# GenomicBreeding/GenomicBreedingModels.jl

Measured on AMD Instinct MI355X. Metric: GRM+GBLUP genotype-cells/s (n x p), higher is better.
Workload: dtype f64

## Files before the change

### genomicbreedingmodels.jl_amd/csrc/chol.hip

```cpp
#include <cstdlib>
#include <string>

#include "chol_device.h"

namespace gbm {

constexpr int NB = kCholNB;
constexpr int MAXRHS = 63;

int launch_chol_update(double* G, int64_t ldg, int64_t k0, int64_t nb, int64_t gdim, double* Ld, double* Dinv,
                       int32_t* info, int64_t next_k0, int rank, int nranks, hipStream_t s, int64_t col_lo = 0,
                       int64_t col_hi = INT64_MAX, int64_t row_lo = 0, int64_t row_hi = INT64_MAX);
int launch_chol_row_update(double* G, int64_t ldg, int64_t k0, int kch, int64_t gdim, double* Ld, double* Dinv,
                           int32_t* info, hipStream_t s, ColKeep keep = ColKeep{});
int64_t chol_small_lim();
void chol_refresh_tuning();
int64_t chol_flow_flag_bytes(int64_t gdim);
bool chol_flow_enabled(int64_t npad);
int launch_chol_flow(double* G, int64_t ldg, int64_t gdim, double* Ld, double* Dinv, void* flag_block, int32_t* info,
                     hipStream_t s);

__global__ void __launch_bounds__(256) prepare_v_kernel(double* __restrict__ G, int64_t ld, int64_t n,
                                                        int64_t npad, int64_t gdim, double inv_q,
                                                        const int64_t* __restrict__ q_dev, double lambda,
// ... 199 lines not shown
    if (area && j == c) {
#pragma unroll
      for (int m = 0; m < 2; m++)
#pragma unroll
        for (int q = 0; q < 2; q++)
#pragma unroll
          for (int r = 0; r < 4; r++) {
            int64_t row, col;
            quad(m, q, r, row, col);
            G[(r0 + row) * ld + jx + col] = accd[m][q][r];
            Us[row * PS + col] = accd[m][q][r];
          }
      __syncthreads();
      const int bad = factor_diag_block(Us, rinv, tid);
      if (tid == 0 && bad >= 0) atomicCAS(info, 0, (int32_t)(r0 + bad + 1));
      const __amdgpu_buffer_rsrc_t rL = wt_rsrc(Ld + r0 * CNB, CNB * CNB * 8);
      const __amdgpu_buffer_rsrc_t rD = wt_rsrc(Dinv + (r0 / 16) * 256, 1024 * 8);
      store_factor_with(
          Us, rinv, tid, [&](int e, wt_d2 v) { wt_st2(rL, (uint32_t)(e * 8), v); },
          [&](int e, double x) { wt_st1(rD, (uint32_t)(e * 8), x); });
      publish_flag(&prog[c], j + 1, tid);
      break;
    }
    {
      const double* src = G + r0 * ld + jx;
#pragma unroll
      for (int m = 0; m < 2; m++)
#pragma unroll
        for (int q = 0; q < 2; q++)
#pragma unroll
          for (int r = 0; r < 4; r++) {
            int64_t row, col;
            quad(m, q, r, row, col);
            acc[m][q][r] = src[row * ld + col];
          }
    }
    int seen = j == 0 ? 1 : 0;
    auto need = [&](int32_t v) -> bool {
      if (seen >= v) return true;
      __syncthreads();
      if (tid == 0) {
        s_ok = wait_flag<false>(&prog[j], v, info) ? 1 : 0;
        s_seen = __hip_atomic_load(&prog[j], __ATOMIC_RELAXED, __HIP_MEMORY_SCOPE_AGENT);
      }
      __syncthreads();
      seen = s_seen;
      return s_ok != 0;
    };
    if (j > 0) {
      d16 va, vb;
      auto load_step = [&](int i) {
        const __amdgpu_buffer_rsrc_t rk = wt_rsrc(G + (k0 + (int64_t)i * CNB) * ld, slab);
#pragma unroll
        for (int e = 0; e < 8; e++) {
          const int64_t rowoff = (int64_t)(lrow + 8 * e) * ld;
          const wt_d2 x = wt_ld2(rk, (uint32_t)((rowoff + r0 + lcol) * 8));
          const wt_d2 y = wt_ld2(rk, (uint32_t)((rowoff + jx + lcol) * 8));
          va[2 * e] = x.x;
          va[2 * e + 1] = x.y;
          vb[2 * e] = y.x;
          vb[2 * e + 1] = y.y;
        }
      };
      if (!need(1)) return;
      load_step(0);
      for (int i = 0; i < j; i++) {
        if (i > 0) __syncthreads();
#pragma unroll
        for (int e = 0; e < 8; e++) {
          *reinterpret_cast<wt_d2*>(&As[(lrow + 8 * e) * PS + lcol]) = (wt_d2){va[2 * e], va[2 * e + 1]};
          *reinterpret_cast<wt_d2*>(&Bs[(lrow + 8 * e) * PS + lcol]) = (wt_d2){vb[2 * e], vb[2 * e + 1]};
        }
        __syncthreads();
        if (i + 1 < j) {
          if (!need(i + 2)) return;
          load_step(i + 1);
        }
#pragma unroll
        for (int ks = 0; ks < 16; ks++) {
          double af[2], bf[2];
#pragma unroll
          for (int m = 0; m < 2; m++) af[m] = -As[(ks * 4 + fr) * PS + wm * 32 + m * 16 + fc];
#pragma unroll
          for (int q = 0; q < 2; q++) bf[q] = Bs[(ks * 4 + fr) * PS + wn * 32 + q * 16 + fc];
#pragma unroll
          for (int m = 0; m < 2; m++)
#pragma unroll
            for (int q = 0; q < 2; q++) acc[m][q] = __builtin_amdgcn_mfma_f64_16x16x4f64(af[m], bf[q], acc[m][q], 0, 0, 0);
        }
      }
      if (!need(j + 1)) return;
    }
    __syncthreads();
    double di[16];
#pragma unroll
    for (int m = 0; m < 2; m++)
#pragma unroll
      for (int q = 0; q < 2; q++)
#pragma unroll
        for (int r = 0; r < 4; r++) {
          int64_t row, col;
          quad(m, q, r, row, col);
          X[row * PS + col] = acc[m][q][r];
        }
    {
      const __amdgpu_buffer_rsrc_t rL = wt_rsrc(Ld + r0 * CNB, CNB * CNB * 8);
      const __amdgpu_buffer_rsrc_t rD = wt_rsrc(Dinv + (r0 / 16) * 256, 1024 * 8);
      wt_d2 u[8];
#pragma unroll
      for (int k = 0; k < 8; k++) u[k] = wt_ld2(rL, (uint32_t)((2 * tid + 512 * k) * 8));
#pragma unroll
      for (int rb = 0; rb < 4; rb++)
#pragma unroll
        for (int ks = 0; ks < 4; ks++) di[rb * 4 + ks] = wt_ld1(rD, (uint32_t)((rb * 256 + (ks * 4 + fr) * 16 + fc) * 8));
#pragma unroll
      for (int k = 0; k < 8; k++) {
        const int e = 2 * tid + 512 * k;
        *reinterpret_cast<wt_d2*>(&Us[(e >> 6) * PS + (e & 63)]) = u[k];
      }
    }
    __syncthreads();
    panel_chunk_solve(X, Us, [&](int rb, int ks) { return di[rb * 4 + ks]; }, lane, wave);
    __syncthreads();
#pragma unroll
    for (int e = 0; e < 8; e++) {
      const int row = lrow + 8 * e;
      wt_st2(rrow, (uint32_t)(((int64_t)row * ld + jx + lcol) * 8), *reinterpret_cast<const wt_d2*>(&X[row * PS + lcol]));
    }
#pragma unroll
    for (int e = 0; e < 8; e++) {
      const int row = lrow + 8 * e;
      *reinterpret_cast<double2*>(G + (jx + row) * ld + r0 + lcol) = make_double2(X[lcol * PS + row], X[(lcol + 1) * PS + row]);
    }
    if (area) {
#pragma unroll
      for (int ks = 0; ks < 16; ks++) {
        double af[2], bf[2];
#pragma unroll
        for (int m = 0; m < 2; m++) af[m] = -X[(ks * 4 + fr) * PS + wm * 32 + m * 16 + fc];
#pragma unroll
        for (int q = 0; q < 2; q++) bf[q] = X[(ks * 4 + fr) * PS + wn * 32 + q * 16 + fc];
#pragma unroll
        for (int m = 0; m < 2; m++)
#pragma unroll
          for (int q = 0; q < 2; q++) accd[m][q] = __builtin_amdgcn_mfma_f64_16x16x4f64(af[m], bf[q], accd[m][q], 0, 0, 0);
      }
      publish_flag(&prog[c], j + 1, tid);
    } else {
      __syncthreads();
    }
  }
}

__global__ void __launch_bounds__(64) diag_inverse_kernel(const double* __restrict__ Ld, double* __restrict__ Linv) {
  __shared__ double Ub[NB][NB + 1];
  const int lane = threadIdx.x;
  const int64_t b0 = (int64_t)blockIdx.x * NB;
  for (int r = 0; r < NB; r++) Ub[r][lane] = Ld[(b0 + r) * NB + lane];
  __syncthreads();
  double x[NB];
#pragma unroll
  for (int i = NB - 1; i >= 0; i--) {
    double p0 = 0.0, p1 = 0.0, p2 = 0.0, p3 = 0.0;
#pragma unroll
    for (int k = i + 1; k < NB; k += 4) {
      p0 = fma(Ub[i][k], x[k], p0);
      if (k + 1 < NB) p1 = fma(Ub[i][k + 1], x[k + 1], p1);
      if (k + 2 < NB) p2 = fma(Ub[i][k + 2], x[k + 2], p2);
      if (k + 3 < NB) p3 = fma(Ub[i][k + 3], x[k + 3], p3);
    }
    x[i] = (i <= lane) ? (((lane == i) ? 1.0 : 0.0) - ((p0 + p1) + (p2 + p3))) * rcp_nr(Ub[i][i]) : 0.0;
  }
#pragma unroll
  for (int i = 0; i < NB; i++) Linv[(b0 + i) * NB + lane] = x[i];
}

__global__ void __launch_bounds__(256) gls_mu_kernel(const double* __restrict__ G, int64_t ld, int64_t npad,
                                                     int64_t nrhs, double* __restrict__ W, int64_t lda,
                                                     double* __restrict__ mu, int32_t* __restrict__ flags) {
  const int64_t t = blockIdx.y;
  const double c11 = -G[npad * ld + npad];
  const double c1y = -G[npad * ld + npad + 1 + t];
  const double m = c1y / c11;
  if (blockIdx.x == 0 && threadIdx.x == 0) mu[t] = m;
  if (t == 0)
    for (int64_t i = (int64_t)blockIdx.x * 256 + threadIdx.x; i < npad / NB; i += (int64_t)gridDim.x * 256) flags[i] = 0;
  for (int64_t i = (int64_t)blockIdx.x * 256 + threadIdx.x; i < lda; i += (int64_t)gridDim.x * 256)
    W[t * lda + i] = i < npad ? G[(npad + 1 + t) * ld + i] - m * G[npad * ld + i] : 0.0;
}

__global__ void __launch_bounds__(256) gblup_terms_kernel(const double* __restrict__ G, int64_t ld, int64_t npad,
                                                          int64_t nrhs, const double* __restrict__ Ld,
                                                          double* __restrict__ terms) {
  __shared__ double red[256];
  double sacc = 0.0;
  for (int64_t r = threadIdx.x; r < npad; r += 256) sacc += log(Ld[r * NB + (r % NB)]);
  red[threadIdx.x] = sacc;
  __syncthreads();
  for (int w = 128; w > 0; w >>= 1) {
    if ((int)threadIdx.x < w) red[threadIdx.x] += red[threadIdx.x + w];
    __syncthreads();
  }
  if (threadIdx.x == 0) {
    terms[0] = 2.0 * red[0];
    terms[1] = -G[npad * ld + npad];
  }
  for (int64_t t = threadIdx.x; t < nrhs; t += 256) {
    terms[2 + 2 * t] = -G[npad * ld + npad + 1 + t];
    terms[3 + 2 * t] = -G[(npad + 1 + t) * ld + npad + 1 + t];
  }
}

constexpr int RC = 4;

__global__ void __launch_bounds__(256) back_solve_kernel(const double* __restrict__ G, int64_t ld,
                                                         const double* __restrict__ Linv, int64_t nb,
                                                         const double* __restrict__ W, double* A,
                                                         int64_t lda, int64_t nrhs, int32_t* __restrict__ flags,
                                                         int32_t* __restrict__ info) {
  __shared__ double part[4][RC][NB];
  __shared__ double rl[RC][NB];
  __shared__ double ah[RC][NB];
  __shared__ int ok_s;
  const int tid = threadIdx.x, lane = tid & 63, wave = tid >> 6;
  const int64_t bh = nb - 1 - 2 * (int64_t)blockIdx.x, bl = bh - 1;
  const bool lo = bl >= 0;
  const int64_t h0 = bh * NB, l0 = bl * NB;
  const int j0 = wave * 16;
  const int64_t a_bytes = nrhs * lda * 8;
  const __amdgpu_buffer_rsrc_t rA =
      __builtin_amdgcn_make_buffer_rsrc(A, (short)0, (int)(a_bytes < 0x7fffffff ? a_bytes : 0x7fffffff), 0x00020000);
  double uh[16], ul[16], lb[16];
#pragma unroll
  for (int jj = 0; jj < 16; jj++) {
    uh[jj] = Linv[(h0 + lane) * NB + j0 + jj];
    ul[jj] = lo ? Linv[(l0 + lane) * NB + j0 + jj] : 0.0;
    lb[jj] = lo ? G[(h0 + j0 + jj) * ld + l0 + lane] : 0.0;
  }
  if (tid == 0) ok_s = 1;
  int32_t pass = 0;
  auto solve_block = [&](int64_t b0, const double (&ui)[16], const double (&acc)[RC], const double (&w)[RC], int tc,
                         int64_t t0, double (*out)[NB]) {
#pragma unroll
    for (int t = 0; t < RC; t++) part[wave][t][lane] = acc[t];
    lds_sync();
    if (wave == 0)
#pragma unroll
      for (int t = 0; t < RC; t++)
        if (t < tc) rl[t][lane] = w[t] - (((part[0][t][lane] + part[1][t][lane]) + part[2][t][lane]) + part[3][t][lane]);
    lds_sync();
    for (int t = 0; t < tc; t++) {
      double s = 0.0;
#pragma unroll
      for (int jj = 0; jj < 16; jj++) s = fma(ui[jj], rl[t][j0 + jj], s);
      part[wave][t][lane] = s;
    }
    lds_sync();
    if (wave == 0)
      for (int t = 0; t < tc; t++) {
        const double v = ((part[0][t][lane] + part[1][t][lane]) + part[2][t][lane]) + part[3][t][lane];
        st_agent(A + (t0 + t) * lda + b0 + lane, v);
        if (out) out[t][lane] = v;
      }
  };
  for (int64_t t0 = 0; t0 < nrhs; t0 += RC) {
    pass++;
    const int tc = (int)(nrhs - t0 < RC ? nrhs - t0 : RC);
    double acch[RC] = {0.0, 0.0, 0.0, 0.0}, accl[RC] = {0.0, 0.0, 0.0, 0.0};
    double wh[RC] = {0.0, 0.0, 0.0, 0.0}, wl[RC] = {0.0, 0.0, 0.0, 0.0};
    if (wave == 0)
#pragma unroll
      for (int t = 0; t < RC; t++)
        if (t < tc) {
          wh[t] = W[(t0 + t) * lda + h0 + lane];
          if (lo) wl[t] = W[(t0 + t) * lda + l0 + lane];
        }
    bool ok = true;
    for (int64_t c = nb - 1; c > bh && ok; c--) {
      double lh[16], ll[16];
      const double* lp = G + (c * NB + j0) * ld + lane;
#pragma unroll
      for (int jj = 0; jj < 16; jj++) {
        lh[jj] = lp[(int64_t)jj * ld + h0];
        ll[jj] = lo ? lp[(int64_t)jj * ld + l0] : 0.0;
      }
      if (lane == 0) ok = wait_flag<false>(&flags[c], pass, info);
      ok = __builtin_amdgcn_readfirstlane((int)ok) != 0;
      __builtin_amdgcn_fence(__ATOMIC_ACQUIRE, "wavefront");
      for (int t = 0; t < tc; t++) {
        const uint32_t voff = (uint32_t)(((t0 + t) * lda + c * NB + j0) * 8);
        double av[16];
#pragma unroll
        for (int jj = 0; jj < 16; jj++)
          av[jj] = __builtin_bit_cast(double, __builtin_amdgcn_raw_buffer_load_b64(rA, (int)(voff + jj * 8), 0, 16));
        double sh = 0.0, sl = 0.0;
#pragma unroll
        for (int jj = 0; jj < 16; jj++) {
          sh = fma(lh[jj], av[jj], sh);
          sl = fma(ll[jj], av[jj], sl);
        }
        acch[t] += sh;
        accl[t] += sl;
      }
    }
    if (!ok) ok_s = 0;
    solve_block(h0, uh, acch, wh, tc, t0, lo ? ah : nullptr);
    publish_flag(&flags[bh], pass, tid);
    if (lo) {
      for (int t = 0; t < tc; t++) {
        double sl = 0.0;
#pragma unroll
        for (int jj = 0; jj < 16; jj++) sl = fma(lb[jj], ah[t][j0 + jj], sl);
        accl[t] += sl;
      }
      lds_sync();
      solve_block(l0, ul, accl, wl, tc, t0, nullptr);
      publish_flag(&flags[bl], pass, tid);
    }
    if (!ok_s) return;
    lds_sync();
  }
}

constexpr int WPA = CNB + 4;
__global__ void __launch_bounds__(512) whiten_rows_kernel(const double* __restrict__ G, int64_t ldg,
                                                          const double* __restrict__ Linv, int64_t nb, double* R,
                                                          int64_t ldr, int64_t rows) {
  __shared__ __attribute__((aligned(16))) double As[2][CNB * WPA];
  __shared__ __attribute__((aligned(16))) double Bs[2][CNB * PS];
  const int tid = threadIdx.x, lane = tid & 63, wave = tid >> 6;
  const int wm = wave >> 2, wn = wave & 3, fr = lane >> 4, fc = lane & 15;
  const int64_t r0 = (int64_t)blockIdx.x * CNB;
  const int lrow = tid >> 5, lcol = 2 * (tid & 31);
  const int cw = wn * 16 + fc;
  typedef double d8 __attribute__((ext_vector_type(8)));
  for (int64_t k = 0; k < nb; k++) {
    d4 acc[2];
#pragma unroll
    for (int m = 0; m < 2; m++)
#pragma unroll
      for (int r = 0; r < 4; r++) {
        const int64_t row = r0 + wm * 32 + m * 16 + fr + 4 * r;
        acc[m][r] = row < rows ? R[row * ldr + k * CNB + cw] : 0.0;
      }
    d8 va0, vb0, va1, vb1;
    auto load_step = [&](int64_t m, d8& va, d8& vb) {
#pragma unroll
      for (int e = 0; e < 4; e++) {
        const int64_t row = r0 + lrow + 16 * e;
        double2 x = make_double2(0.0, 0.0);
        if (row < rows) x = *reinterpret_cast<const double2*>(R + row * ldr + m * CNB + lcol);
        const double2 y = *reinterpret_cast<const double2*>(G + (m * CNB + lrow + 16 * e) * ldg + k * CNB + lcol);
        va[2 * e] = x.x;
        va[2 * e + 1] = x.y;
        vb[2 * e] = y.x;
        vb[2 * e + 1] = y.y;
      }
    };
    auto stage = [&](int buf, const d8& va, const d8& vb) {
#pragma unroll
      for (int e = 0; e < 4; e++) {
        *reinterpret_cast<double2*>(&As[buf][(lrow + 16 * e) * WPA + lcol]) = make_double2(va[2 * e], va[2 * e + 1]);
        *reinterpret_cast<double2*>(&Bs[buf][(lrow + 16 * e) * PS + lcol]) = make_double2(vb[2 * e], vb[2 * e + 1]);
      }
    };
    auto step = [&](int64_t m, int buf, d8& na, d8& nb_) {
      const double* Am = As[buf];
      const double* Bm = Bs[buf];
#pragma unroll
      for (int ks = 0; ks < 16; ks++) {
        const double bf = Bm[(ks * 4 + fr) * PS + cw];
#pragma unroll
        for (int mm = 0; mm < 2; mm++) {
          const double af = -Am[(wm * 32 + mm * 16 + fc) * WPA + ks * 4 + fr];
          acc[mm] = __builtin_amdgcn_mfma_f64_16x16x4f64(af, bf, acc[mm], 0, 0, 0);
        }
      }
      if (m + 1 < k) {
        stage(buf ^ 1, na, nb_);
        if (m + 3 < k) load_step(m + 3, na, nb_);
      }
      __syncthreads();
    };
    if (k > 0) {
      load_step(0, va0, vb0);
      if (k > 1) load_step(1, va1, vb1);
      stage(0, va0, vb0);
      if (k > 2) load_step(2, va0, vb0);
      __syncthreads();
    }
    for (int64_t m = 0; m < k; m += 2) {
      step(m, 0, va1, vb1);
      if (m + 1 < k) step(m + 1, 1, va0, vb0);
    }
#pragma unroll
    for (int m = 0; m < 2; m++)
#pragma unroll
      for (int r = 0; r < 4; r++) As[0][(wm * 32 + m * 16 + fr + 4 * r) * WPA + cw] = acc[m][r];
#pragma unroll
    for (int e = 0; e < 4; e++)
      *reinterpret_cast<double2*>(&Bs[0][(lrow + 16 * e) * PS + lcol]) =
          *reinterpret_cast<const double2*>(Linv + (k * CNB + lrow + 16 * e) * CNB + lcol);
    __syncthreads();
    d4 out[2];
#pragma unroll
    for (int m = 0; m < 2; m++) out[m] = (d4){0.0, 0.0, 0.0, 0.0};
#pragma unroll
    for (int ks = 0; ks < 16; ks++) {
      const double bf = Bs[0][(ks * 4 + fr) * PS + cw];
#pragma unroll
      for (int mm = 0; mm < 2; mm++) {
        const double af = As[0][(wm * 32 + mm * 16 + fc) * WPA + ks * 4 + fr];
        out[mm] = __builtin_amdgcn_mfma_f64_16x16x4f64(af, bf, out[mm], 0, 0, 0);
      }
    }
#pragma unroll
    for (int m = 0; m < 2; m++)
#pragma unroll
      for (int r = 0; r < 4; r++) {
        const int64_t row = r0 + wm * 32 + m * 16 + fr + 4 * r;
        if (row < rows) R[row * ldr + k * CNB + cw] = out[m][r];
      }
    __builtin_amdgcn_s_waitcnt(0);
    __syncthreads();
  }
}

__global__ void __launch_bounds__(256) gebv_kernel(const double* __restrict__ Y, int64_t ldy, int64_t n,
                                                   const double* __restrict__ A, double* __restrict__ gebv,
                                                   int64_t lda, const double* __restrict__ mu, double lambda) {
  const int64_t t = blockIdx.y;
  const double m = mu[t];
  for (int64_t i = (int64_t)blockIdx.x * 256 + threadIdx.x; i < lda; i += (int64_t)gridDim.x * 256)
    gebv[t * lda + i] = i < n ? m + (Y[t * ldy + i] - m) - lambda * A[t * lda + i] : 0.0;
}

}

using namespace gbm;

extern "C" int64_t gbm_dev_npad(int64_t n) { return npad_of(n); }
extern "C" int64_t gbm_dev_gdim(int64_t n) { return gdim_of(n); }
static int64_t flow_block_offset(int64_t n) { return round_up(npad_of(n) * (2 * NB + 16) + npad_of(n) / NB / 2 + 1, 2); }
static int64_t solve_ws_doubles(int64_t n) { return flow_block_offset(n) + chol_flow_flag_bytes(gdim_of(n)) / 8; }
extern "C" int64_t gbm_dev_solve_workspace(int64_t n, int64_t nrhs) {
  (void)nrhs;
  return solve_ws_doubles(n) * (int64_t)sizeof(double);
}

namespace {

struct SolveWs {
  double *Ld, *Linv, *Dinv;
  int32_t* flags;
  void* flow;
};
SolveWs solve_ws(void* workspace, int64_t npad) {
  SolveWs w;
  w.Ld = (double*)workspace;
  w.Linv = w.Ld + npad * NB;
  w.Dinv = w.Linv + npad * NB;
  w.flags = reinterpret_cast<int32_t*>(w.Dinv + npad * 16);
  w.flow = (double*)workspace + flow_block_offset(npad);
  return w;
}

int check_solve_args(const double* G, int64_t ldg, int64_t n, const int32_t* info, const void* workspace,
                     int64_t ws_bytes, const char* who) {
  if (!G || !info || n < 1 || ldg < gdim_of(n) || (ldg & 1) || ((uintptr_t)G & 15))
    return fail(GBM_E_ARG, std::string(who) + ": bad arguments (G 16-byte aligned, even ldg >= gdim(n))");
  if (!workspace || ws_bytes < solve_ws_doubles(n) * (int64_t)sizeof(double) || ((uintptr_t)workspace & 15))
    return fail(GBM_E_ARG, std::string(who) + ": workspace too small (see gbm_dev_solve_workspace)");
  return GBM_OK;
}

static int64_t tail_flow_rows(int64_t npad) {
  const char* e = ::gbm::knob("GBM_CHOL_TAIL_FLOW");
  if (e) return (int64_t)atoll(e);
  return npad > 12288 ? 8192 : 0;
}
static bool tail_flow_at(int64_t kb, int64_t npad, int64_t gdim) {
  return kb > 0 && kb < npad / NB && gdim - kb * NB <= tail_flow_rows(npad);
}

int group_size(int64_t kb, int64_t nb, int64_t gdim) {
  if (tail_flow_at(kb, nb * NB, gdim)) return (int)(nb - kb);
  auto lim = [](const char* name, int64_t dflt) {
    const char* e = ::gbm::knob(name);
    return e ? (int64_t)atoll(e) : dflt;
  };
  const int64_t g4 = lim("GBM_CHOL_G4_LIM", 8192), g8 = lim("GBM_CHOL_G8_LIM", 8192),
                g16 = lim("GBM_CHOL_G16_LIM", 16384);
  const int64_t k0 = kb * NB;
  if (g16 >= 0 && kb + 16 < nb && gdim - (k0 + 16 * NB) > g16) return 16;
  if (g8 >= 0 && kb + 8 < nb && gdim - (k0 + 8 * NB) > g8) return 8;
  if (g4 >= 0 && kb + 4 < nb && gdim - (k0 + 4 * NB) > g4) return 4;
  if (kb + 2 < nb && gdim - (k0 + 2 * NB) > chol_small_lim()) return 2;
  return 1;
}

int solve_prepare(double* G, int64_t ldg, int64_t n, double inv_q, const int64_t* q_dev, double lambda,
                  const double* Y, int64_t ldy, int64_t nrhs, int32_t* info, void* workspace, hipStream_t s,
                  bool factor_first = true, ColKeep keep = ColKeep{}) {
  const int64_t npad = npad_of(n), gdim = gdim_of(n);
  const SolveWs w = solve_ws(workspace, npad);
  chol_refresh_tuning();
  prepare_v_kernel<<<(unsigned)gdim, 256, 0, s>>>(G, ldg, n, npad, gdim, inv_q, q_dev, lambda, Y, ldy, nrhs, info,
                                                  keep);
  GBM_LAUNCH_CHECK();
  if (!factor_first) return GBM_OK;
  factor_diag_kernel<<<1, 256, 0, s>>>(G, ldg, 0, w.Ld, w.Dinv, info);
  GBM_LAUNCH_CHECK();
  return GBM_OK;
}

static bool group_kernel_enabled() {
  const char* e = ::gbm::knob("GBM_CHOL_GROUP_KERNEL");
  return !e || atoi(e) != 0;
}

int solve_group_panels(double* G, int64_t ldg, int64_t n, int64_t kb, ColKeep keep, int32_t* info, void* workspace,
                       hipStream_t s, int64_t* g_out) {
  const int64_t npad = npad_of(n), gdim = gdim_of(n), nb = npad / NB;
  const SolveWs w = solve_ws(workspace, npad);
  const int64_t k0 = kb * NB;
  if (tail_flow_at(kb, npad, gdim))
    return fail(GBM_E_ARG, "gbm_dev_chol_group_panels: the dataflow tail (GBM_CHOL_TAIL_FLOW) runs as gbm_dev_chol_group");
  const int g = group_size(kb, nb, gdim);
  if (keep.nranks > 1) {
    if (g < 2 || (k0 % 128) != 0)
      return fail(GBM_E_ARG, "gbm_dev_chol_group_panels: a distributed step needs a panel group of >= 2 panels on a "
                             "128-row boundary (finish the tail with gbm_dev_chol_group, nranks = 1)");
    keep.keep_hi = k0 + g * NB;
    keep.rhs0 = npad;
  }
  if (g_out) *g_out = g;
  if (g > 1 && group_kernel_enabled()) {
    GroupCols gc;
    gc.g = g;
    gc.nranks = keep.nranks;
    gc.a0 = kb + g;
    gc.rhs0 = npad / NB;
    gc.n_rhs = (gdim - npad) / NB;
    if (keep.nranks == 1) {
      gc.n_own = npad / NB - gc.a0;
    } else {
      const int64_t R = keep.nranks, J0 = gc.a0 / 2;
      if ((gc.a0 & 1) != 0) return fail(GBM_E_ARG, "gbm_dev_chol_group_panels: odd panel group in a distributed step");
      gc.J_first = J0 + ((keep.rank - J0) % R + R) % R;
      for (int64_t J = gc.J_first; 2 * J < npad / NB; J += R) gc.n_own += (2 * J + 1 < npad / NB) ? 2 : 1;
    }
    if ((int64_t)(CNB + 1) * ldg * 8 > 0x7fffffff)
      return fail(GBM_E_ARG, "chol_group_kernel: ldg too large for 32-bit buffer offsets");
    int32_t* prog = reinterpret_cast<int32_t*>(w.flow);
    GBM_HIP_TRY(hipMemsetAsync(prog, 0, (size_t)g * sizeof(int32_t), s));
    const int64_t nwg = (g - 1) + gc.n_own + gc.n_rhs;
    chol_group_kernel<<<(unsigned)nwg, 256, 0, s>>>(G, ldg, k0, gc, w.Ld, w.Dinv, prog, info);
    GBM_LAUNCH_CHECK();
    return GBM_OK;
  }
  auto panel = [&](int64_t k) {
    const int64_t chunks = (gdim - k) / NB - 1;
    chol_panel_kernel<<<(unsigned)chunks, 256, 0, s>>>(G, ldg, k, w.Ld, w.Dinv, keep);
    return hipGetLastError() == hipSuccess;
  };
  if (!panel(k0)) return fail(GBM_E_HIP, "chol_panel_kernel launch failed");
  for (int j = 1; j < g; j++) {
    GBM_TRY(launch_chol_row_update(G, ldg, k0, j, gdim, w.Ld, w.Dinv, info, s, keep));
    if (!panel(k0 + j * NB)) return fail(GBM_E_HIP, "chol_panel_kernel launch failed");
  }
  return GBM_OK;
}

int solve_group_update(double* G, int64_t ldg, int64_t n, int64_t kb, int rank, int nranks, int32_t* info,
                       void* workspace, hipStream_t s, int64_t col_lo = 0, int64_t col_hi = INT64_MAX,
                       int64_t row_lo = 0, int64_t row_hi = INT64_MAX) {
  const int64_t npad = npad_of(n), gdim = gdim_of(n), nb = npad / NB;
  const SolveWs w = solve_ws(workspace, npad);
  const int64_t k0 = kb * NB;
  if (tail_flow_at(kb, npad, gdim))
    return fail(GBM_E_ARG, "gbm_dev_chol_group_update: the dataflow tail (GBM_CHOL_TAIL_FLOW) runs as gbm_dev_chol_group");
  const int g = group_size(kb, nb, gdim);
  const int64_t next = kb + g < nb ? k0 + g * NB : -1;
  if (g > 1)
    return launch_chol_update(G, ldg, k0, g * NB, gdim, w.Ld, w.Dinv, info, next, rank, nranks, s, col_lo, col_hi,
                              row_lo, row_hi);
  if (nranks > 1) return fail(GBM_E_ARG, "gbm_dev_chol_group_update: single-panel steps are not distributed");
  return launch_chol_update(G, ldg, k0, NB, gdim, w.Ld, w.Dinv, info, next, 0, 1, s);
}

int solve_group(double* G, int64_t ldg, int64_t n, int64_t kb, int32_t* info, void* workspace, hipStream_t s,
                int64_t* g_out) {
  const int64_t npad = npad_of(n), gdim = gdim_of(n);
  if (tail_flow_at(kb, npad, gdim)) {
    const SolveWs w = solve_ws(workspace, npad);
    const int64_t k0 = kb * NB;
    if (g_out) *g_out = npad / NB - kb;
    return launch_chol_flow(G + k0 * ldg + k0, ldg, gdim - k0, w.Ld + k0 * CNB, w.Dinv + (k0 / 16) * 256, w.flow,
                            info, s);
  }
  GBM_TRY(solve_group_panels(G, ldg, n, kb, ColKeep{}, info, workspace, s, g_out));
  return solve_group_update(G, ldg, n, kb, 0, 1, info, workspace, s);
}

int solve_finish(double* G, int64_t ldg, int64_t n, const double* Y, int64_t ldy, int64_t nrhs, double lambda,
                 double* A_out, double* gebv, int64_t lda, double* mu, int32_t* info, void* workspace, hipStream_t s) {
  const int64_t npad = npad_of(n), nb = npad / NB;
  const SolveWs w = solve_ws(workspace, npad);
  diag_inverse_kernel<<<(unsigned)nb, 64, 0, s>>>(w.Ld, w.Linv);
  GBM_LAUNCH_CHECK();
  const unsigned gx = (unsigned)((lda + 255) / 256 < 1024 ? (lda + 255) / 256 : 1024);
  gls_mu_kernel<<<dim3(gx, (unsigned)nrhs), 256, 0, s>>>(G, ldg, npad, nrhs, gebv, lda, mu, w.flags);
  GBM_LAUNCH_CHECK();
  back_solve_kernel<<<(unsigned)((nb + 1) / 2), 256, 0, s>>>(G, ldg, w.Linv, nb, gebv, A_out, lda, nrhs, w.flags, info);
  GBM_LAUNCH_CHECK();
  gebv_kernel<<<dim3(gx, (unsigned)nrhs), 256, 0, s>>>(Y, ldy, n, A_out, gebv, lda, mu, lambda);
  GBM_LAUNCH_CHECK();
  return GBM_OK;
}

void strip_geometry(int64_t n, int64_t kb, int64_t rows64, int nranks, int64_t& r0, int64_t& rows, int64_t& J0,
                    int64_t& Jend, int64_t& cnt, bool area = false) {
  r0 = kb * NB;
  rows = rows64 * NB;
  J0 = r0 / 128;
  Jend = area ? (r0 + rows + 127) / 128 : npad_of(n) / 128;
  cnt = Jend > J0 ? (Jend - J0 + nranks - 1) / nranks : 0;
}

}

extern "C" int gbm_dev_gblup_solve(double* G, int64_t ldg, int64_t n, double inv_q, const int64_t* q_dev,
                                   double lambda, const double* Y, int64_t ldy, int64_t nrhs, double* A_out,
                                   double* gebv, int64_t lda, double* mu, int32_t* info, void* workspace,
                                   int64_t ws_bytes, void* stream) {
  const int64_t npad = npad_of(n);
  if (!Y || !A_out || !gebv || !mu || ldy < n || lda < npad || nrhs < 1 || nrhs > MAXRHS || !(lambda > 0.0) ||
      !(q_dev || inv_q > 0.0))
    return fail(GBM_E_ARG, "gbm_dev_gblup_solve: bad arguments (need ldg >= gdim(n), lda >= npad(n), "
                           "1 <= nrhs <= 63, lambda > 0, inv_q > 0)");
  GBM_TRY(check_solve_args(G, ldg, n, info, workspace, ws_bytes, "gbm_dev_gblup_solve"));
  hipStream_t s = (hipStream_t)stream;
  if (chol_flow_enabled(npad)) {
    GBM_TRY(solve_prepare(G, ldg, n, inv_q, q_dev, lambda, Y, ldy, nrhs, info, workspace, s, false));
    const SolveWs w = solve_ws(workspace, npad);
    GBM_TRY(launch_chol_flow(G, ldg, gdim_of(n), w.Ld, w.Dinv, w.flow, info, s));
    return solve_finish(G, ldg, n, Y, ldy, nrhs, lambda, A_out, gebv, lda, mu, info, workspace, s);
  }
  GBM_TRY(solve_prepare(G, ldg, n, inv_q, q_dev, lambda, Y, ldy, nrhs, info, workspace, s));
  const int64_t nb = npad / NB;
  for (int64_t kb = 0; kb < nb;) {
    int64_t g = 1;
    GBM_TRY(solve_group(G, ldg, n, kb, info, workspace, s, &g));
    kb += g;
  }
  return solve_finish(G, ldg, n, Y, ldy, nrhs, lambda, A_out, gebv, lda, mu, info, workspace, s);
}

extern "C" int gbm_dev_chol_prepare(double* G, int64_t ldg, int64_t n, double inv_q, const int64_t* q_dev,
                                    double lambda, const double* Y, int64_t ldy, int64_t nrhs, int32_t* info,
                                    void* workspace, int64_t ws_bytes, void* stream) {
  if (!Y || ldy < n || nrhs < 1 || nrhs > MAXRHS || !(lambda > 0.0) || !(q_dev || inv_q > 0.0))
    return fail(GBM_E_ARG, "gbm_dev_chol_prepare: bad arguments");
  GBM_TRY(check_solve_args(G, ldg, n, info, workspace, ws_bytes, "gbm_dev_chol_prepare"));
  return solve_prepare(G, ldg, n, inv_q, q_dev, lambda, Y, ldy, nrhs, info, workspace, (hipStream_t)stream);
}

extern "C" int gbm_dev_chol_prepare_cols(double* G, int64_t ldg, int64_t n, double inv_q, const int64_t* q_dev,
                                         double lambda, const double* Y, int64_t ldy, int64_t nrhs, int rank,
                                         int nranks, int32_t* info, void* workspace, int64_t ws_bytes, void* stream) {
  if (!Y || ldy < n || nrhs < 1 || nrhs > MAXRHS || !(lambda > 0.0) || !(q_dev || inv_q > 0.0) || nranks < 1 ||
      rank < 0 || rank >= nranks)
    return fail(GBM_E_ARG, "gbm_dev_chol_prepare_cols: bad arguments");
  GBM_TRY(check_solve_args(G, ldg, n, info, workspace, ws_bytes, "gbm_dev_chol_prepare_cols"));
  ColKeep keep;
  keep.rank = rank;
  keep.nranks = nranks;
  if (nranks > 1) {
    chol_refresh_tuning();
    keep.keep_hi = (int64_t)group_size(0, npad_of(n) / NB, gdim_of(n)) * NB;
    keep.rhs0 = npad_of(n);
  }
  return solve_prepare(G, ldg, n, inv_q, q_dev, lambda, Y, ldy, nrhs, info, workspace, (hipStream_t)stream, true, keep);
}

extern "C" int64_t gbm_dev_chol_group_size(int64_t n, int64_t kb) {
  const int64_t nb = npad_of(n) / NB;
  if (kb < 0 || kb >= nb) return 0;
  chol_refresh_tuning();
  return group_size(kb, nb, gdim_of(n));
}

extern "C" int gbm_dev_chol_group(double* G, int64_t ldg, int64_t n, int64_t kb, int rank, int nranks, int32_t* info,
                                  void* workspace, int64_t ws_bytes, void* stream) {
  GBM_TRY(check_solve_args(G, ldg, n, info, workspace, ws_bytes, "gbm_dev_chol_group"));
  if (kb < 0 || kb >= npad_of(n) / NB || nranks != 1 || rank != 0)
    return fail(GBM_E_ARG, "gbm_dev_chol_group: one rank only (rank 0 of 1); a distributed step is "
                           "gbm_dev_chol_group_panels + row exchange + gbm_dev_chol_group_update");
  return solve_group(G, ldg, n, kb, info, workspace, (hipStream_t)stream, nullptr);
}

extern "C" int gbm_dev_chol_group_panels(double* G, int64_t ldg, int64_t n, int64_t kb, int rank, int nranks,
                                         int32_t* info, void* workspace, int64_t ws_bytes, void* stream) {
  GBM_TRY(check_solve_args(G, ldg, n, info, workspace, ws_bytes, "gbm_dev_chol_group_panels"));
  if (kb < 0 || kb >= npad_of(n) / NB || nranks < 1 || rank < 0 || rank >= nranks)
    return fail(GBM_E_ARG, "gbm_dev_chol_group_panels: bad step or rank");
  ColKeep keep;
  keep.rank = rank;
  keep.nranks = nranks;
  return solve_group_panels(G, ldg, n, kb, keep, info, workspace, (hipStream_t)stream, nullptr);
}

extern "C" int gbm_dev_chol_group_update(double* G, int64_t ldg, int64_t n, int64_t kb, int rank, int nranks,
                                         int32_t* info, void* workspace, int64_t ws_bytes, void* stream) {
  GBM_TRY(check_solve_args(G, ldg, n, info, workspace, ws_bytes, "gbm_dev_chol_group_update"));
  if (kb < 0 || kb >= npad_of(n) / NB || nranks < 1 || rank < 0 || rank >= nranks)
    return fail(GBM_E_ARG, "gbm_dev_chol_group_update: bad step or rank");
  return solve_group_update(G, ldg, n, kb, rank, nranks, info, workspace, (hipStream_t)stream);
}

extern "C" int gbm_dev_chol_group_update_cols(double* G, int64_t ldg, int64_t n, int64_t kb, int rank, int nranks,
                                              int64_t col_lo, int64_t col_hi, int32_t* info, void* workspace,
                                              int64_t ws_bytes, void* stream) {
  GBM_TRY(check_solve_args(G, ldg, n, info, workspace, ws_bytes, "gbm_dev_chol_group_update_cols"));
  if (kb < 0 || kb >= npad_of(n) / NB || nranks < 2 || rank < 0 || rank >= nranks || col_lo < 0 || col_hi < col_lo)
    return fail(GBM_E_ARG, "gbm_dev_chol_group_update_cols: bad step, rank (nranks >= 2) or column range");
  return solve_group_update(G, ldg, n, kb, rank, nranks, info, workspace, (hipStream_t)stream, col_lo, col_hi);
}

extern "C" int gbm_dev_chol_group_update_tiles(double* G, int64_t ldg, int64_t n, int64_t kb, int rank, int nranks,
                                               int64_t row_lo, int64_t row_hi, int64_t col_lo, int64_t col_hi,
                                               int32_t* info, void* workspace, int64_t ws_bytes, void* stream) {
  GBM_TRY(check_solve_args(G, ldg, n, info, workspace, ws_bytes, "gbm_dev_chol_group_update_tiles"));
  if (kb < 0 || kb >= npad_of(n) / NB || nranks < 2 || rank < 0 || rank >= nranks || col_lo < 0 || col_hi < col_lo ||
      row_lo < 0 || row_hi < row_lo)
    return fail(GBM_E_ARG, "gbm_dev_chol_group_update_tiles: bad step, rank (nranks >= 2), row or column range");
  return solve_group_update(G, ldg, n, kb, rank, nranks, info, workspace, (hipStream_t)stream, col_lo, col_hi, row_lo,
                            row_hi);
}

extern "C" int gbm_dev_chol_factor_diag(double* G, int64_t ldg, int64_t n, int64_t kb, int32_t* info, void* workspace,
                                        int64_t ws_bytes, void* stream) {
  GBM_TRY(check_solve_args(G, ldg, n, info, workspace, ws_bytes, "gbm_dev_chol_factor_diag"));
  if (kb < 0 || kb >= npad_of(n) / NB) return fail(GBM_E_ARG, "gbm_dev_chol_factor_diag: bad step");
  const SolveWs w = solve_ws(workspace, npad_of(n));
  factor_diag_kernel<<<1, 256, 0, (hipStream_t)stream>>>(G, ldg, kb * NB, w.Ld, w.Dinv, info);
  GBM_LAUNCH_CHECK();
  return GBM_OK;
}

extern "C" int64_t gbm_dev_chol_strip_doubles(int64_t n, int64_t kb, int64_t rows64, int nranks) {
  if (nranks < 1 || kb < 0 || rows64 < 1) return 0;
  int64_t r0, rows, J0, Jend, cnt;
  strip_geometry(n, kb, rows64, nranks, r0, rows, J0, Jend, cnt);
  return cnt * rows * 128;
}

static int strip_launch(double* G, int64_t ldg, int64_t n, int64_t kb, int64_t rows64, int rank, int nranks,
                        double* buf, int unpack, hipStream_t s, bool area = false) {
  if (!G || !buf || n < 1 || ldg < gdim_of(n) || kb < 0 || rows64 < 1 || (kb * NB) % 128 != 0 || nranks < 1 ||
      rank < 0 || rank >= nranks || (kb + rows64) * NB > npad_of(n))
    return fail(GBM_E_ARG, "gbm_dev_chol_strip_pack/unpack: bad arguments (strip rows inside [0, npad), "
                           "starting on a 128-row boundary)");
  if (area && (rows64 & 1))
    return fail(GBM_E_ARG, "gbm_dev_chol_area_pack/unpack: the area must end on a 128-row boundary");
  int64_t r0, rows, J0, Jend, cnt;
  strip_geometry(n, kb, rows64, nranks, r0, rows, J0, Jend, cnt, area);
  if (cnt == 0) return GBM_OK;
  if (cnt > 65535 || nranks > 65535) return fail(GBM_E_ARG, "gbm_dev_chol_strip_*: too many tiles for the grid");
  const dim3 grid((unsigned)((rows + 3) / 4), (unsigned)cnt, (unsigned)(unpack ? nranks : 1));
// ... 94 lines not shown
```

Before: 12.14 billion.

## Fuse GLS/GEBV into back-solve, use sentinel sync, parallelize diagonal inverse

The back-solve now polls A itself for a NaN-pattern sentinel, which the diagonal-inverse kernel pre-fills, instead of waiting on per-block flags. It also folds the gls_mu and gebv kernels into back_solve, computing mu, W and GEBV inline, which removes two launches and the W round trip. A 256-thread diagonal-inverse variant spreads each column across four lanes and combines them with DPP quad shuffles. All three paths are on by default behind env knobs; the sentinel scheme adds spin-polling on data and could misfire if a real value matches the bit pattern.

Result: no change. 12.17 billion, median of 5 (+0.2%).

```diff
diff --git a/genomicbreedingmodels.jl_amd/csrc/chol.hip b/genomicbreedingmodels.jl_amd/csrc/chol.hip
--- a/genomicbreedingmodels.jl_amd/csrc/chol.hip
+++ b/genomicbreedingmodels.jl_amd/csrc/chol.hip
@@ -375,10 +375,20 @@
   }
 }
 
-__global__ void __launch_bounds__(64) diag_inverse_kernel(const double* __restrict__ Ld, double* __restrict__ Linv) {
+constexpr uint64_t kASentinel = ~(uint64_t)0;
+
+__device__ __forceinline__ void fill_a_sentinel(double* __restrict__ A, int64_t lda, int64_t nrhs, int64_t b0) {
+  if (!A) return;
+  for (int64_t e = threadIdx.x; e < nrhs * NB; e += blockDim.x)
+    A[(e / NB) * lda + b0 + (e % NB)] = __builtin_bit_cast(double, kASentinel);
+}
+
+__global__ void __launch_bounds__(64) diag_inverse_kernel(const double* __restrict__ Ld, double* __restrict__ Linv,
+                                                          double* __restrict__ A, int64_t lda, int64_t nrhs) {
   __shared__ double Ub[NB][NB + 1];
   const int lane = threadIdx.x;
   const int64_t b0 = (int64_t)blockIdx.x * NB;
+  fill_a_sentinel(A, lda, nrhs, b0);
   for (int r = 0; r < NB; r++) Ub[r][lane] = Ld[(b0 + r) * NB + lane];
   __syncthreads();
   double x[NB];
@@ -396,6 +406,54 @@
   }
 #pragma unroll
   for (int i = 0; i < NB; i++) Linv[(b0 + i) * NB + lane] = x[i];
+}
+
+template <int S>
+__device__ __forceinline__ double quad_lane(double x) {
+  union {
+    double d;
+    int i[2];
+  } u;
+  u.d = x;
+  u.i[0] = __builtin_amdgcn_mov_dpp(u.i[0], S * 0x55, 0xf, 0xf, true);
+  u.i[1] = __builtin_amdgcn_mov_dpp(u.i[1], S * 0x55, 0xf, 0xf, true);
+  return u.d;
+}
+template <int R>
+__device__ __forceinline__ void diag_inv4_row(const double (*Ub)[NB + 1], const double* rinv, int m, int l, int j,
+                                              double (&xl)[NB / 4]) {
+  const int i = 4 * m + R;
+  double p = 0.0;
+  if (l > R) p = fma(Ub[i][4 * m + l], xl[m], p);
+#pragma unroll
+  for (int mm = m + 1; mm < NB / 4; mm++) p = fma(Ub[i][4 * mm + l], xl[mm], p);
+  const double p0 = quad_lane<(R + 1) & 3>(p), p1 = quad_lane<(R + 2) & 3>(p), p2 = quad_lane<(R + 3) & 3>(p),
+               p3 = quad_lane<R>(p);
+  const double xi = (i <= j) ? (((j == i) ? 1.0 : 0.0) - ((p0 + p1) + (p2 + p3))) * rinv[i] : 0.0;
+  if (l == R) xl[m] = xi;
+}
+__global__ void __launch_bounds__(256) diag_inverse4_kernel(const double* __restrict__ Ld, double* __restrict__ Linv,
+                                                            double* __restrict__ A, int64_t lda, int64_t nrhs) {
+  __shared__ double Ub[NB][NB + 1];
+  __shared__ double rinv[NB];
+  const int tid = threadIdx.x, j = tid >> 2, l = tid & 3;
+  const int64_t b0 = (int64_t)blockIdx.x * NB;
+  fill_a_sentinel(A, lda, nrhs, b0);
+  for (int r = tid >> 6; r < NB; r += 4) Ub[r][tid & 63] = Ld[(b0 + r) * NB + (tid & 63)];
+  if (tid < NB) rinv[tid] = rcp_nr(Ld[(b0 + tid) * NB + tid]);
+  __syncthreads();
+  double xl[NB / 4];
+#pragma unroll
+  for (int m = 0; m < NB / 4; m++) xl[m] = 0.0;
+#pragma unroll
+  for (int m = NB / 4 - 1; m >= 0; m--) {
+    diag_inv4_row<3>(Ub, rinv, m, l, j, xl);
+    diag_inv4_row<2>(Ub, rinv, m, l, j, xl);
+    diag_inv4_row<1>(Ub, rinv, m, l, j, xl);
+    diag_inv4_row<0>(Ub, rinv, m, l, j, xl);
+  }
+#pragma unroll
+  for (int m = 0; m < NB / 4; m++) Linv[(b0 + 4 * m + l) * NB + j] = xl[m];
 }
 
 __global__ void __launch_bounds__(256) gls_mu_kernel(const double* __restrict__ G, int64_t ld, int64_t npad,
@@ -409,7 +467,7 @@
   if (t == 0)
     for (int64_t i = (int64_t)blockIdx.x * 256 + threadIdx.x; i < npad / NB; i += (int64_t)gridDim.x * 256) flags[i] = 0;
   for (int64_t i = (int64_t)blockIdx.x * 256 + threadIdx.x; i < lda; i += (int64_t)gridDim.x * 256)
-    W[t * lda + i] = i < npad ? G[(npad + 1 + t) * ld + i] - m * G[npad * ld + i] : 0.0;
+    W[t * lda + i] = i < npad ? fma(-m, G[npad * ld + i], G[(npad + 1 + t) * ld + i]) : 0.0;
 }
 
 __global__ void __launch_bounds__(256) gblup_terms_kernel(const double* __restrict__ G, int64_t ld, int64_t npad,
@@ -436,14 +494,22 @@
 
 constexpr int RC = 4;
 
+struct BackFold {
+  const double* Y;
+  int64_t ldy, n;
+  double lambda;
+  double *gebv, *mu;
+};
+template <bool kSentinel, bool kFold>
 __global__ void __launch_bounds__(256) back_solve_kernel(const double* __restrict__ G, int64_t ld,
                                                          const double* __restrict__ Linv, int64_t nb,
                                                          const double* __restrict__ W, double* A,
                                                          int64_t lda, int64_t nrhs, int32_t* __restrict__ flags,
-                                                         int32_t* __restrict__ info) {
+                                                         int32_t* __restrict__ info, BackFold f) {
   __shared__ double part[4][RC][NB];
   __shared__ double rl[RC][NB];
   __shared__ double ah[RC][NB];
+  __shared__ double gm_s[RC], gy_s[2][RC][NB];
   __shared__ int ok_s;
   const int tid = threadIdx.x, lane = tid & 63, wave = tid >> 6;
   const int64_t bh = nb - 1 - 2 * (int64_t)blockIdx.x, bl = bh - 1;
@@ -451,6 +517,15 @@
   const int64_t h0 = bh * NB, l0 = bl * NB;
   const int j0 = wave * 16;
   const int64_t a_bytes = nrhs * lda * 8;
+  const int64_t npad = nb * NB;
+  if constexpr (kFold) {
+    if (blockIdx.x == 0) {
+      const double c11 = -G[npad * ld + npad];
+      for (int64_t t = tid; t < nrhs; t += 256) f.mu[t] = -G[npad * ld + npad + 1 + t] / c11;
+      for (int64_t e = tid; e < nrhs * (lda - npad); e += 256)
+        f.gebv[(e / (lda - npad)) * lda + npad + e % (lda - npad)] = 0.0;
+    }
+  }
   const __amdgpu_buffer_rsrc_t rA =
       __builtin_amdgcn_make_buffer_rsrc(A, (short)0, (int)(a_bytes < 0x7fffffff ? a_bytes : 0x7fffffff), 0x00020000);
   double uh[16], ul[16], lb[16];
@@ -463,7 +538,7 @@
   if (tid == 0) ok_s = 1;
   int32_t pass = 0;
   auto solve_block = [&](int64_t b0, const double (&ui)[16], const double (&acc)[RC], const double (&w)[RC], int tc,
-                         int64_t t0, double (*out)[NB]) {
+                         int64_t t0, double (*out)[NB], const double (*gy)[NB]) {
 #pragma unroll
     for (int t = 0; t < RC; t++) part[wave][t][lane] = acc[t];
     lds_sync();
@@ -479,12 +554,20 @@
       part[wave][t][lane] = s;
     }
     lds_sync();
-    if (wave == 0)
+    if (wave == 0) {
+      const bool gave_up = kSentinel && !ok_s;
       for (int t = 0; t < tc; t++) {
-        const double v = ((part[0][t][lane] + part[1][t][lane]) + part[2][t][lane]) + part[3][t][lane];
+        double v = ((part[0][t][lane] + part[1][t][lane]) + part[2][t][lane]) + part[3][t][lane];
+        if constexpr (kSentinel) {
+          if (gave_up) v = 0.0;
+          if (__builtin_bit_cast(uint64_t, v) == kASentinel) v = __builtin_nan("");
+        }
         st_agent(A + (t0 + t) * lda + b0 + lane, v);
         if (out) out[t][lane] = v;
-      }
+        if constexpr (kFold)
+          f.gebv[(t0 + t) * lda + b0 + lane] = b0 + lane < f.n ? fma(-f.lambda, v, gm_s[t] + (gy[t][lane] - gm_s[t])) : 0.0;
+      }
+    }
   };
   for (int64_t t0 = 0; t0 < nrhs; t0 += RC) {
     pass++;
@@ -495,8 +578,19 @@
 #pragma unroll
       for (int t = 0; t < RC; t++)
         if (t < tc) {
-          wh[t] = W[(t0 + t) * lda + h0 + lane];
-          if (lo) wl[t] = W[(t0 + t) * lda + l0 + lane];
+          if constexpr (kFold) {
+            const double c11 = -G[npad * ld + npad];
+            const double c1y = -G[npad * ld + npad + 1 + t0 + t];
+            const double m = c1y / c11;
+            if (lane == 0) gm_s[t] = m;
+            wh[t] = fma(-m, G[npad * ld + h0 + lane], G[(npad + 1 + t0 + t) * ld + h0 + lane]);
+            if (lo) wl[t] = fma(-m, G[npad * ld + l0 + lane], G[(npad + 1 + t0 + t) * ld + l0 + lane]);
+            gy_s[0][t][lane] = h0 + lane < f.n ? f.Y[(t0 + t) * f.ldy + h0 + lane] : 0.0;
+            gy_s[1][t][lane] = lo && l0 + lane < f.n ? f.Y[(t0 + t) * f.ldy + l0 + lane] : 0.0;
+          } else {
+            wh[t] = W[(t0 + t) * lda + h0 + lane];
+            if (lo) wl[t] = W[(t0 + t) * lda + l0 + lane];
+          }
         }
     bool ok = true;
     for (int64_t c = nb - 1; c > bh && ok; c--) {
@@ -507,15 +601,34 @@
         lh[jj] = lp[(int64_t)jj * ld + h0];
         ll[jj] = lo ? lp[(int64_t)jj * ld + l0] : 0.0;
       }
-      if (lane == 0) ok = wait_flag<false>(&flags[c], pass, info);
-      ok = __builtin_amdgcn_readfirstlane((int)ok) != 0;
+      if constexpr (!kSentinel) {
+        if (lane == 0) ok = wait_flag<false>(&flags[c], pass, info);
+        ok = __builtin_amdgcn_readfirstlane((int)ok) != 0;
+      }
       __builtin_amdgcn_fence(__ATOMIC_ACQUIRE, "wavefront");
-      for (int t = 0; t < tc; t++) {
+      for (int t = 0; t < tc && ok; t++) {
         const uint32_t voff = (uint32_t)(((t0 + t) * lda + c * NB + j0) * 8);
         double av[16];
-#pragma unroll
-        for (int jj = 0; jj < 16; jj++)
-          av[jj] = __builtin_bit_cast(double, __builtin_amdgcn_raw_buffer_load_b64(rA, (int)(voff + jj * 8), 0, 16));
+        for (int it = 0;; it++) {
+#pragma unroll
+          for (int jj = 0; jj < 16; jj++)
+            av[jj] = __builtin_bit_cast(double, __builtin_amdgcn_raw_buffer_load_b64(rA, (int)(voff + jj * 8), 0, 16));
+          if constexpr (!kSentinel) break;
+          bool pending = false;
+#pragma unroll
+          for (int jj = 0; jj < 16; jj++) pending |= __builtin_bit_cast(uint64_t, av[jj]) == kASentinel;
+          if (!pending) break;
+          if ((it & 255) == 255) {
+            if (__hip_atomic_load(info, __ATOMIC_RELAXED, __HIP_MEMORY_SCOPE_AGENT) < 0) ok = false;
+            if (ok && it > 1 << 22) {
+              __hip_atomic_store(info, -1, __ATOMIC_RELAXED, __HIP_MEMORY_SCOPE_AGENT);
+              ok = false;
+            }
+            if (!ok) break;
+          }
+          __builtin_amdgcn_s_sleep(2);
+          __builtin_amdgcn_fence(__ATOMIC_ACQUIRE, "wavefront");
+        }
         double sh = 0.0, sl = 0.0;
 #pragma unroll
         for (int jj = 0; jj < 16; jj++) {
@@ -527,8 +640,11 @@
       }
     }
     if (!ok) ok_s = 0;
-    solve_block(h0, uh, acch, wh, tc, t0, lo ? ah : nullptr);
-    publish_flag(&flags[bh], pass, tid);
+    solve_block(h0, uh, acch, wh, tc, t0, lo ? ah : nullptr, gy_s[0]);
+    if constexpr (kSentinel)
+      lds_sync();
+    else
+      publish_flag(&flags[bh], pass, tid);
     if (lo) {
       for (int t = 0; t < tc; t++) {
         double sl = 0.0;
@@ -537,8 +653,8 @@
         accl[t] += sl;
       }
       lds_sync();
-      solve_block(l0, ul, accl, wl, tc, t0, nullptr);
-      publish_flag(&flags[bl], pass, tid);
+      solve_block(l0, ul, accl, wl, tc, t0, nullptr, gy_s[1]);
+      if constexpr (!kSentinel) publish_flag(&flags[bl], pass, tid);
     }
     if (!ok_s) return;
     lds_sync();
@@ -655,7 +771,7 @@
   const int64_t t = blockIdx.y;
   const double m = mu[t];
   for (int64_t i = (int64_t)blockIdx.x * 256 + threadIdx.x; i < lda; i += (int64_t)gridDim.x * 256)
-    gebv[t * lda + i] = i < n ? m + (Y[t * ldy + i] - m) - lambda * A[t * lda + i] : 0.0;
+    gebv[t * lda + i] = i < n ? fma(-lambda, A[t * lda + i], m + (Y[t * ldy + i] - m)) : 0.0;
 }
 
 }
@@ -830,15 +946,42 @@
                  double* A_out, double* gebv, int64_t lda, double* mu, int32_t* info, void* workspace, hipStream_t s) {
   const int64_t npad = npad_of(n), nb = npad / NB;
   const SolveWs w = solve_ws(workspace, npad);
-  diag_inverse_kernel<<<(unsigned)nb, 64, 0, s>>>(w.Ld, w.Linv);
+  auto on = [](const char* name) {
+    const char* e = ::gbm::knob(name);
+    return !e || !*e || atoi(e) != 0;
+  };
+  const bool sentinel = on("GBM_BACK_SENTINEL"), fold = on("GBM_BACK_FOLD"), inv4 = on("GBM_DIAG_INV4");
+  double* fill = sentinel ? A_out : nullptr;
+  if (inv4)
+    diag_inverse4_kernel<<<(unsigned)nb, 256, 0, s>>>(w.Ld, w.Linv, fill, lda, nrhs);
+  else
+    diag_inverse_kernel<<<(unsigned)nb, 64, 0, s>>>(w.Ld, w.Linv, fill, lda, nrhs);
   GBM_LAUNCH_CHECK();
   const unsigned gx = (unsigned)((lda + 255) / 256 < 1024 ? (lda + 255) / 256 : 1024);
-  gls_mu_kernel<<<dim3(gx, (unsigned)nrhs), 256, 0, s>>>(G, ldg, npad, nrhs, gebv, lda, mu, w.flags);
+  if (!fold) {
+    gls_mu_kernel<<<dim3(gx, (unsigned)nrhs), 256, 0, s>>>(G, ldg, npad, nrhs, gebv, lda, mu, w.flags);
+    GBM_LAUNCH_CHECK();
+  } else if (!sentinel) {
+    GBM_HIP_TRY(hipMemsetAsync(w.flags, 0, (size_t)nb * sizeof(int32_t), s));
+  }
+  const BackFold f{Y, ldy, n, lambda, gebv, mu};
+  const unsigned bg = (unsigned)((nb + 1) / 2);
+#define GBM_BACK_SOLVE(S, F) \
+  back_solve_kernel<S, F><<<bg, 256, 0, s>>>(G, ldg, w.Linv, nb, (F) ? nullptr : gebv, A_out, lda, nrhs, w.flags, info, f)
+  if (sentinel && fold)
+    GBM_BACK_SOLVE(true, true);
+  else if (sentinel)
+    GBM_BACK_SOLVE(true, false);
+  else if (fold)
+    GBM_BACK_SOLVE(false, true);
+  else
+    GBM_BACK_SOLVE(false, false);
+#undef GBM_BACK_SOLVE
   GBM_LAUNCH_CHECK();
-  back_solve_kernel<<<(unsigned)((nb + 1) / 2), 256, 0, s>>>(G, ldg, w.Linv, nb, gebv, A_out, lda, nrhs, w.flags, info);
-  GBM_LAUNCH_CHECK();
-  gebv_kernel<<<dim3(gx, (unsigned)nrhs), 256, 0, s>>>(Y, ldy, n, A_out, gebv, lda, mu, lambda);
-  GBM_LAUNCH_CHECK();
+  if (!fold) {
+    gebv_kernel<<<dim3(gx, (unsigned)nrhs), 256, 0, s>>>(Y, ldy, n, A_out, gebv, lda, mu, lambda);
+    GBM_LAUNCH_CHECK();
+  }
   return GBM_OK;
 }
 
```
